# Alex-McAvoy/Light-Graph-Convolutional-Recommendation-Algorithm-based-on-Hybrid-Spreading

Hardware: AMD Instinct MI355X
Metric: propagation edges/sec + full-catalog top-K recs/sec, 1/2/4/8 MI355X (higher is better)
Workload: dtype f32; 1 GPU; c5-d64; users=1000000, items=1000000, interactions=100000000, directed_nnz=200000000, dim=64, layers=3, parallelism=row-shard x1 + RCCL all-gather per layer

## Files before the change

### light-graph-convolutional-recommendation-algorithm-based-on-hybrid-spreading_amd/csrc/spread_tiled.hip

```cpp
#include <stdio.h>
#include <stdlib.h>

#include "common.h"

#ifndef LG_REFERENCE_PATHS
#define LG_REFERENCE_PATHS 0
#endif
#if LG_REFERENCE_PATHS
#include "lgcnhs_ref.h"
#endif

namespace lg {

typedef float f32x4 __attribute__((ext_vector_type(4)));

constexpr uint32_t kHdrV = 0x80000000u;
constexpr uint32_t kHdrOvf = 0x40000000u;
constexpr uint32_t kHdrSlow = 0x20000000u;
constexpr uint32_t kHdrPtr = 0x1FFFFFFFu;
constexpr uint32_t kEntV = 0x80000000u;
constexpr uint32_t kRunDense = 0x80000000u;
constexpr int kLineSlots = 31;
constexpr int kLineEnts = 7;
constexpr int kInvTab = 512;
// ... 948 lines not shown
          while (need) {
            const int u = __ffsll((long long)need) - 1;
            need &= need - 1;
            compact_user(g, u, lim);
          }
        }
      }
    }
  };

  float af0[Q], af1[Q], af2[Q], af3[Q];
  double f0[NG][4], f1[NG][4], f2[NG][4], f3[NG][4];
  load_step(0, af0, f0);
  load_step(16, af1, f1);
  load_step(32, af2, f2);
  for (int it = 0;; it += 64) {
    load_step(it + 48, af3, f3);
    process(it, af0, f0);
    if (it + 16 >= n_cols) break;
    load_step(it + 64, af0, f0);
    process(it + 16, af1, f1);
    if (it + 32 >= n_cols) break;
    load_step(it + 80, af1, f1);
    process(it + 32, af2, f2);
    if (it + 48 >= n_cols) break;
    load_step(it + 96, af2, f2);
    process(it + 48, af3, f3);
    if (it + 64 >= n_cols) break;
  }

  wave_sync();
#pragma unroll
  for (int g = 0; g < NG; ++g) {
    for (int u = 0; u < 16; ++u) {
      const int64_t r = ubase + g * 16 + u;
      if (r >= n_rows) break;
      if (!__shfl((int)dirty[g], u)) continue;
      compact_user(g, u, lim_end);
      const int nc = __shfl(cnt[g], u);
      for (int e = lane; e < k; e += 64) {
        const double v = e < nc ? cs[wave][g][u][e] : neg_inf<double>();
        const bool ok = e < nc && v != neg_inf<double>();
        io_val[r * k + e] = ok ? v : neg_inf<double>();
        io_idx[r * k + e] = ok ? ci[wave][g][u][e] : -1;
      }
      wave_sync();
    }
  }
}

#endif

constexpr int MODE_F = 0, MODE_TOPK = 1;
constexpr int kWalkQ = 8;
constexpr int kBatchRows = 8 * kWalkQ;
constexpr int kOvfList = kBatchRows > 64 ? kBatchRows : 64;
constexpr int kDecodePhase = 4;
constexpr int kQPre = 8;
static_assert(kWalkQ % kDecodePhase == 0, "decode phase must divide the batch's line loads");

struct WalkArgs {
  const int64_t *user_rowptr;
  const int32_t *user_items;
  const double *ra_edge;
  int64_t n_users;
  const uint4 *lines;
  const uint4 *ovf;
  int32_t null_row;
  int32_t item_begin, tile, width;
  const double *rbeta;
  const double *g_inv;
  double *F;
  int64_t ldf;
  const float *eu, *ei;
  const float *gb;
  int32_t nch;
  const uint8_t *qb;
  int32_t qstride;
  const int64_t *ex_rowptr;
  const int32_t *ex_col;
  int64_t *ex_cur;
  int k, first;
  double *io_val;
  int64_t *io_idx;
};

__host__ __device__ constexpr int acc_cols(int tile) { return (tile + 511) / 512 * 512; }

template <int MODE, int D, int M>
__host__ __device__ constexpr size_t walk_wave_bytes(int tile) {
  return ((size_t)acc_cols(tile) * 8 + (size_t)kOvfList * 12 + 15) & ~(size_t)15;
}
__host__ __device__ constexpr size_t walk_shared_bytes(int tile) {
  return (size_t)kInvTab * 8 + 16 * 8 + (size_t)((tile + 1) & ~1) * 8 + 64 * 8;
}


typedef __attribute__((address_space(3))) double lds_f64;
__device__ __forceinline__ double slot_inv_fast(uint32_t s) {
  return *(const lds_f64 *)(uintptr_t)(s >> 13);
}
__device__ __forceinline__ void slot_add_nobranch(uint32_t acc_base, uint32_t dummy, uint32_t s,
                                                  double v) {
  uint32_t addr;
  asm("v_mad_u32_u16 %0, %1, 8, %2" : "=v"(addr) : "v"(s), "v"(acc_base));
  addr = s ? addr : dummy;
  __hip_atomic_fetch_add((lds_f64 *)(uintptr_t)addr, v, __ATOMIC_RELAXED,
                         __HIP_MEMORY_SCOPE_WORKGROUP);
}

__device__ __forceinline__ double slot_inv(uint32_t s, const double *s_inv,
                                           const double *__restrict__ g_inv) {
  const uint32_t c = s >> 16;
  const bool far = c >= (uint32_t)kInvTab;
  const double inv = s_inv[far ? 0u : c];
  if (__builtin_expect(__ballot(far) != 0, 0)) {
    const double g = __builtin_nontemporal_load(g_inv + (far ? c : 0u));
    return far ? g : inv;
  }
  return inv;
}

__device__ __forceinline__ void add_unit(double *acc, uint4 w, bool head, double ra,
                                         const double *s_inv, const double *__restrict__ g_inv) {
  const bool isv = !head && (w.x & kEntV);
  const uint32_t sx = head ? 0u : w.x;
  const uint32_t py = isv ? 0u : w.y, pz = isv ? 0u : w.z, pw = isv ? 0u : w.w;
  const double i0 = slot_inv(isv ? 0u : sx, s_inv, g_inv);
  const double v0 = (isv ? __hiloint2double((int)w.z, (int)w.y) : i0) * ra;
  const double v1 = slot_inv(py, s_inv, g_inv) * ra;
  const double v2 = slot_inv(pz, s_inv, g_inv) * ra;
  const double v3 = slot_inv(pw, s_inv, g_inv) * ra;
  if (sx) lds_add(acc, sx & 0xFFFFu, v0);
  if (py) lds_add(acc, py & 0xFFFFu, v1);
  if (pz) lds_add(acc, pz & 0xFFFFu, v2);
  if (pw) lds_add(acc, pw & 0xFFFFu, v3);
}

__device__ __forceinline__ void add_unit_v(double *acc, uint4 w, double ra) {
  if (w.x & kEntV) lds_add(acc, w.x & 0xFFFFu, __hiloint2double((int)w.z, (int)w.y) * ra);
}
__device__ __forceinline__ void add_unit_d(double *acc, uint4 w, int q, double ra) {
  const double a = __hiloint2double((int)w.y, (int)w.x), b = __hiloint2double((int)w.w, (int)w.z);
  if (a != 0.0) lds_add(acc, (uint32_t)(2 * q), a * ra);
  if (b != 0.0) lds_add(acc, (uint32_t)(2 * q + 1), b * ra);
}

__device__ __forceinline__ void add_slot_fast(double *acc, uint32_t s, double ra,
                                              const double *s_inv) {
  const double inv = s_inv[s >> 16];
  if (s) lds_add(acc, s & 0xFFFFu, inv * ra);
}

struct Batch {
  int32_t u, r0, r1, e;
  bool first;
  int32_t xc, xh;
};

struct UState {
  int lid0, lid1;
  double lv0, lv1;
  float gb;
  uint32_t q[kQPre];
  int32_t xw;
};

template <int MODE, int D, int M, bool SEED = false>
__global__ __launch_bounds__(512) void k_tile_walk(WalkArgs a) {
  constexpr int Q = kWalkQ;
  extern __shared__ double lds[];
  const int nw = blockDim.x / 64;
  const int wave = __builtin_amdgcn_readfirstlane(threadIdx.x / 64);
  const int lane = lane_id();
  const int gh = lane & 7;
  const int grow = lane >> 3;
  const uint32_t hmask = gh == 0 ? 0u : 0xFFFFFFFFu;
  const int tile = a.tile;
  double *s_inv = lds;
  double *s_red = s_inv + kInvTab;
  double *s_rb = s_red + 16;
  double *s_rbc = s_rb + ((tile + 1) & ~1);
  char *mine = reinterpret_cast<char *>(s_rbc + 64) +
               (size_t)wave * walk_wave_bytes<MODE, D, M>(tile);
  double *acc = reinterpret_cast<double *>(mine);
  const uint32_t acc_base = (uint32_t)(uintptr_t)(lds_f64 *)acc;
  const uint32_t dummy_addr = acc_base + 8u * (uint32_t)(acc_cols(tile) + lane);
  double *ovl_ra = acc + acc_cols(tile);
  uint32_t *ovl_ent = reinterpret_cast<uint32_t *>(ovl_ra + kOvfList);

  for (int c = threadIdx.x; c < kInvTab; c += blockDim.x) s_inv[c] = a.g_inv[c];
  double rmax = 0.0;
  for (int j = threadIdx.x; j < tile; j += blockDim.x) {
    const double rb = j < a.width ? a.rbeta[a.item_begin + j] : 0.0;
    s_rb[j] = rb;
    rmax = fmax(rmax, rb);
  }
#pragma unroll
  for (int o = 32; o > 0; o >>= 1) rmax = fmax(rmax, __shfl_xor(rmax, o));
  if (lane == 0) s_red[wave] = rmax;
  for (int j = lane; j < acc_cols(tile); j += 64) acc[j] = 0.0;
  __syncthreads();
  if (MODE == MODE_TOPK && D > 0) {
    for (int c = wave; 64 * c < tile && c < 64; c += nw) {
      double m = s_rb[64 * c + lane < tile ? 64 * c + lane : 0];
#pragma unroll
      for (int o = 32; o > 0; o >>= 1) m = fmax(m, __shfl_xor(m, o));
      if (lane == 0) s_rbc[c] = m;
    }
    __syncthreads();
  }
  rmax = 0.0;
  for (int w = 0; w < nw; ++w) rmax = fmax(rmax, s_red[w]);
  const double rscale = rmax * (1.0 + 0x1p-50);

  const int64_t G = (int64_t)gridDim.x * nw;
  const int64_t n_users = a.n_users;
  const int64_t u_first = (int64_t)blockIdx.x * nw + wave;
  if (u_first >= n_users) return;

  const bool has_ex = MODE == MODE_TOPK && a.ex_rowptr != nullptr;
  int32_t uq = (int32_t)u_first;
  int32_t pr = 0, px = 0;
  auto pre_load = [&]() __attribute__((always_inline)) {
    const int64_t uu = uq < n_users ? uq : n_users - 1;
    pr = reinterpret_cast<const int32_t *>(a.user_rowptr)[2 * (uu + (lane & 1))];
    if (has_ex) {
      const int64_t *p = (lane & 1) ? a.ex_rowptr + uu + 1 : a.ex_cur + uu;
      px = *reinterpret_cast<const int32_t *>(p);
    }
  };
  pre_load();
  auto new_user = [&]() __attribute__((always_inline)) {
    const int32_t bq = __builtin_amdgcn_readlane(pr, 0), eq = __builtin_amdgcn_readlane(pr, 1);
    const int32_t xcq = has_ex ? __builtin_amdgcn_readlane(px, 0) : 0;
    const int32_t xhq = has_ex ? __builtin_amdgcn_readlane(px, 1) : 0;
    Batch y{uq, bq, bq + kBatchRows < eq ? bq + kBatchRows : eq, eq, true, xcq, xhq};
    uq += (int32_t)G;
    return y;
  };
  const Batch kEnd{(int32_t)n_users, 0, 0, 0, false, 0, 0};
  auto next_batch = [&](const Batch &x) __attribute__((always_inline)) {
    if (x.u >= n_users) return kEnd;
    if (x.r1 < x.e) {
      Batch y{x.u, x.r1, x.r1 + kBatchRows < x.e ? x.r1 + kBatchRows : x.e, x.e, false, x.xc,
              x.xh};
      return y;
    }
    if (x.u + G >= n_users) return kEnd;
    return new_user();
  };
  const __amdgpu_buffer_rsrc_t r_lines = __builtin_amdgcn_make_buffer_rsrc(
      (void *)a.lines, 0, (int)((uint32_t)(a.null_row + 1) * 128u), 0x00020000);
  auto load_ids = [&](const Batch &x, int32_t (&it)[Q]) __attribute__((always_inline)) {
    {
      const __amdgpu_buffer_rsrc_t rs = __builtin_amdgcn_make_buffer_rsrc(
          (void *)(a.user_items + x.r0), 0, (int)((x.r1 - x.r0) * 4), 0x00020000);
#pragma unroll
      for (int q = 0; q < Q; ++q)
        it[q] = (int32_t)__builtin_amdgcn_raw_buffer_load_b32(rs, (uint32_t)(grow * 4 + 32 * q),
                                                              0, 0);
    }
  };
  auto load_rows = [&](const Batch &x, const int32_t (&it)[Q], uint4 (&w)[Q], double (&ra)[Q])
      __attribute__((always_inline)) {
    const int nr = (int)(x.r1 - x.r0);
    const __amdgpu_buffer_rsrc_t rr = __builtin_amdgcn_make_buffer_rsrc(
        (void *)(a.ra_edge + x.r0), 0, nr * 8, 0x00020000);
#pragma unroll
    for (int q = 0; q < Q; ++q) {
      const bool in = 8 * q + grow < nr;
      const uint32_t row = in ? (uint32_t)it[q] : (uint32_t)a.null_row;
      const auto v = __builtin_amdgcn_raw_buffer_load_b128(r_lines, row * 128u + 16u * gh, 0, 0);
      w[q] = uint4{v[0], v[1], v[2], v[3]};
      const auto d = __builtin_amdgcn_raw_buffer_load_b64(rr, (uint32_t)(grow * 8 + 64 * q), 0, 0);
      ra[q] = __builtin_bit_cast(double, d);
    }
  };

  constexpr bool kTwo = M > 2;
  const bool has_qb = MODE == MODE_TOPK && D > 0 && a.qb != nullptr;
  auto load_state = [&](const Batch &x, UState &st) __attribute__((always_inline)) {
    if constexpr (MODE == MODE_TOPK) {
      const int k = a.k;
      const int64_t us = x.u < n_users ? x.u : n_users - 1;
      const int *idx32 = reinterpret_cast<const int *>(a.io_idx);
      const int e0 = lane < k ? lane : k - 1;
      st.lid0 = idx32[2 * (us * k + e0)];
      st.lv0 = a.io_val[us * k + e0];
      if constexpr (kTwo) {
        const int e1 = 64 + lane < k ? 64 + lane : k - 1;
        st.lid1 = idx32[2 * (us * k + e1)];
        st.lv1 = a.io_val[us * k + e1];
      }
      if constexpr (D > 0) {
        st.gb = a.gb[us * a.nch + (lane < a.nch ? lane : 0)];
        const __amdgpu_buffer_rsrc_t rq = __builtin_amdgcn_make_buffer_rsrc(
            has_qb ? (void *)(a.qb + us * a.qstride) : (void *)a.lines, 0,
            has_qb ? a.qstride : 0, 0x00020000);
#pragma unroll
        for (int kk = 0; kk < kQPre; ++kk)
          st.q[kk] = __builtin_amdgcn_raw_buffer_load_b32(rq, (uint32_t)(4 * lane + 256 * kk), 0, 0);
      }
      const int32_t nx = x.xh - x.xc;
      const __amdgpu_buffer_rsrc_t rx = __builtin_amdgcn_make_buffer_rsrc(
          has_ex ? (void *)(a.ex_col + x.xc) : (void *)a.lines, 0,
          has_ex ? (int)(4 * (nx < 64 ? nx : 64)) : 0, 0x00020000);
      st.xw = (int32_t)__builtin_amdgcn_raw_buffer_load_b32(rx, (uint32_t)(4 * lane), 0, 0);
    }
  };

  auto decode = [&](const Batch &x, uint4 (&w)[Q], const double (&ra)[Q])
      __attribute__((always_inline)) {
#ifdef LG_WALK_PROBE
    if (LG_WALK_PROBE == 2) {
      uint32_t h = 0;
#pragma unroll
      for (int q = 0; q < Q; ++q) h ^= w[q].x ^ w[q].y ^ w[q].z ^ w[q].w ^ (uint32_t)ra[q];
      if (h == 0x12345678u && lane == 64) acc[0] = 1.0;
      return;
    }
#endif
    uint32_t hdr = 0;
#pragma unroll
    for (int q = 0; q < Q; ++q) hdr |= w[q].x & ~hmask;
    const bool slow = __ballot(hdr & kHdrSlow) != 0;
    const bool ovf = __ballot(hdr & kHdrOvf) != 0;
    if (!slow) {
      constexpr int H = kDecodePhase;
      const int nr = (int)(x.r1 - x.r0);
#pragma unroll
      for (int q0 = 0; q0 < Q; q0 += H) {
        if (8 * q0 >= nr) break;
        double inv[H][4];
#pragma unroll
        for (int q = 0; q < H; ++q) {
          if (8 * (q0 + q) >= nr) break;
          inv[q][0] = slot_inv_fast(w[q0 + q].x & hmask);
          inv[q][1] = slot_inv_fast(w[q0 + q].y);
          inv[q][2] = slot_inv_fast(w[q0 + q].z);
          inv[q][3] = slot_inv_fast(w[q0 + q].w);
        }
#pragma unroll
        for (int q = 0; q < H; ++q) {
          if (8 * (q0 + q) >= nr) break;
          const uint32_t sv[4] = {w[q0 + q].x & hmask, w[q0 + q].y, w[q0 + q].z, w[q0 + q].w};
#pragma unroll
          for (int t = 0; t < 4; ++t)
            slot_add_nobranch(acc_base, dummy_addr, sv[t], inv[q][t] * ra[q0 + q]);
        }
      }
    } else {
#pragma unroll
      for (int q = 0; q < Q; ++q) add_unit(acc, w[q], gh == 0, ra[q], s_inv, a.g_inv);
    }
    if (ovf) {
      int nov = 0;
#pragma unroll
      for (int q = 0; q < Q; ++q) {
        const bool o = gh == 0 && (w[q].x & kHdrOvf);
        const uint64_t bal = __ballot(o);
        if (o) {
          const int p = nov + __popcll(bal & lanemask_lt());
          ovl_ent[p] = w[q].x & (kHdrPtr | kHdrV);
          ovl_ra[p] = ra[q];
        }
        nov += __popcll(bal);
      }
      wave_sync();
      for (int t0 = 0; t0 < nov; t0 += 4) {
        uint4 y4[4];
        uint32_t ou4[4];
        double r4[4];
        bool v4[4];
#pragma unroll
        for (int j = 0; j < 4; ++j) {
          const bool in = t0 + j < nov;
          const uint32_t e = ovl_ent[in ? t0 + j : t0];
          v4[j] = (e & kHdrV) != 0;
          ou4[j] = e & kHdrPtr;
          r4[j] = ovl_ra[in ? t0 + j : t0];
          y4[j] = a.ovf[(int64_t)ou4[j] + lane];
        }
#pragma unroll
        for (int j = 0; j < 4; ++j) {
          if (t0 + j >= nov) continue;
          const uint32_t n0 = (uint32_t)__shfl((int)y4[j].x, 0);
          const bool dn = (n0 & kRunDense) != 0;
          const uint32_t n = n0 & ~kRunDense;
          if (lane == 0 || (uint32_t)lane > n) y4[j] = uint4{0u, 0u, 0u, 0u};
          if (dn) add_unit_d(acc, y4[j], lane - 1, r4[j]);
          else if (v4[j]) add_unit_v(acc, y4[j], r4[j]);
          else add_unit(acc, y4[j], false, r4[j], s_inv, a.g_inv);
          for (uint32_t c = 64; c <= n; c += 256) {
            uint4 z[4];
#pragma unroll
            for (int p = 0; p < 4; ++p) {
              const uint32_t cc = c + 64 * p + lane;
              z[p] = cc <= n ? a.ovf[(int64_t)ou4[j] + cc] : uint4{0u, 0u, 0u, 0u};
            }
#pragma unroll
            for (int p = 0; p < 4; ++p) {
              if (c + 64 * p > n) break;
              if (dn) add_unit_d(acc, z[p], (int)(c + 64 * p) + lane - 1, r4[j]);
              else if (v4[j]) add_unit_v(acc, z[p], r4[j]);
              else add_unit(acc, z[p], false, r4[j], s_inv, a.g_inv);
            }
          }
        }
      }
      wave_sync();
    }
  };

  auto finish_user = [&](const Batch &x, UState &st) __attribute__((always_inline)) {
    const int64_t u = x.u;
    wave_sync();
#ifdef LG_WALK_PROBE
    if (LG_WALK_PROBE == 1) {
      for (int j = 2 * lane; j < acc_cols(tile); j += 128)
        *reinterpret_cast<double2 *>(acc + j) = double2{0.0, 0.0};
      wave_sync();
      return;
    }
#endif
    if constexpr (MODE == MODE_F) {
      double *row = a.F + u * a.ldf;
      for (int j = lane; j < tile; j += 64) {
        __builtin_nontemporal_store(acc[j] * s_rb[j], row + j);
        acc[j] = 0.0;
      }
    } else {
      const int k = a.k;
      const bool ok0 = !a.first && lane < k && st.lid0 >= 0;
      double L0 = ok0 ? st.lv0 : neg_inf<double>();
      int I0 = ok0 ? st.lid0 : kPadId;
      double L1 = neg_inf<double>();
      int I1 = kPadId;
      if constexpr (kTwo) {
        const bool ok1 = !a.first && 64 + lane < k && st.lid1 >= 0;
        L1 = ok1 ? st.lv1 : neg_inf<double>();
        I1 = ok1 ? st.lid1 : kPadId;
      }
      const float gbv = st.gb;
      uint32_t (&qr)[kQPre] = st.q;
      if (!has_qb) {
#pragma unroll
        for (int kk = 0; kk < kQPre; ++kk) qr[kk] = 0xFFFFFFFFu;
      }
      int64_t xpos = x.xc;
      const int64_t xhi = x.xh;
      int32_t xw = has_ex && xpos + lane < xhi ? st.xw : 0x7fffffff;
      auto kth = [&](double &tv, int &ti) __attribute__((always_inline)) {
        if (!kTwo || k <= 64) {
          tv = __shfl(L0, k - 1);
          ti = __shfl(I0, k - 1);
        } else {
          tv = __shfl(L1, k - 65);
          ti = __shfl(I1, k - 65);
        }
      };
      double tau;
      int tau_id;
      kth(tau, tau_id);
      bool dirty = a.first != 0;
      auto insert1 = [&](double v, int id) __attribute__((always_inline)) {
        if (!before(v, id, tau, tau_id)) return;
        dirty = true;
        int pos = __popcll(__ballot(before(L0, I0, v, id)));
        if constexpr (kTwo) pos += __popcll(__ballot(before(L1, I1, v, id)));
        const double up0 = __shfl_up(L0, 1);
        const int iu0 = __shfl_up(I0, 1);
        if constexpr (kTwo) {
          const double up1 = __shfl_up(L1, 1);
          const int iu1 = __shfl_up(I1, 1);
          const double c0 = __shfl(L0, 63);
          const int ic0 = __shfl(I0, 63);
          const int p1 = 64 + lane;
          const double n1 = p1 > pos ? (lane == 0 ? c0 : up1) : (p1 == pos ? v : L1);
          const int m1 = p1 > pos ? (lane == 0 ? ic0 : iu1) : (p1 == pos ? id : I1);
          L1 = p1 < k ? n1 : neg_inf<double>();
          I1 = p1 < k ? m1 : kPadId;
        }
        L0 = lane > pos ? up0 : (lane == pos ? v : L0);
        I0 = lane > pos ? iu0 : (lane == pos ? id : I0);
        if (lane >= k) { L0 = neg_inf<double>(); I0 = kPadId; }
        kth(tau, tau_id);
      };
      const int32_t lim = a.item_begin + a.width;
      if (has_ex) {
        for (;;) {
          const bool in = xw < lim;
          if (in && xw >= a.item_begin) acc[xw - a.item_begin] = neg_inf<double>();
          const int nin = __popcll(__ballot(in));
          xpos += nin;
          if (nin < 64) break;
          xw = xpos + lane < xhi ? a.ex_col[xpos + lane] : 0x7fffffff;
        }
        if (lane == 0) a.ex_cur[u] = xpos;
      }
      wave_sync();
      int ncand = 0;
      double *cq_f = ovl_ra;
      uint32_t *cq_j = ovl_ent;
      auto flush = [&]() __attribute__((always_inline)) {
#ifdef LG_WALK_PROBE
        if (LG_WALK_PROBE == 3) {
          wave_sync();
          for (int mm = 0; mm < ncand; ++mm) insert1(cq_f[mm], a.item_begin + (int)cq_j[mm]);
          ncand = 0;
          wave_sync();
          return;
        }
#endif
        if constexpr (D > 0) {
          constexpr int Qd = D / 4;
          constexpr int H = Qd < 16 ? Qd : 16;
          wave_sync();
          const int m = lane & 15, g = lane >> 4;
          for (int b0 = 0; b0 < ncand; b0 += 16) {
            const int nb = ncand - b0 < 16 ? ncand - b0 : 16;
            const int ci = b0 + (m < nb ? m : 0);
            const float *ir = a.ei + (int64_t)(a.item_begin + (int)cq_j[ci]) * D + g * Qd;
            const float *ur = a.eu + u * D + g * Qd;
            f32x4 sc4 = f32x4{0.f, 0.f, 0.f, 0.f};
#pragma unroll
            for (int h0 = 0; h0 < Qd; h0 += H) {
              float av[H], bv[H];
              load_frag<H>(ir + h0, av);
              load_frag<H>(ur + h0, bv);
#pragma unroll
              for (int s = 0; s < H; ++s)
                sc4 = __builtin_amdgcn_mfma_f32_16x16x4f32(av[s], bv[s], sc4, 0, 0, 0);
            }
            for (int mm = 0; mm < nb; ++mm) {
              const float e = (mm & 3) == 0 ? sc4[0] : (mm & 3) == 1 ? sc4[1]
                            : (mm & 3) == 2 ? sc4[2] : sc4[3];
              const float sc = __shfl(e, 16 * (mm >> 2));
              insert1((double)sc * cq_f[b0 + mm], a.item_begin + (int)cq_j[b0 + mm]);
            }
          }
          ncand = 0;
          wave_sync();
        }
      };
      double thr_s = tau / rscale;
      double sc_v = 0.0, bq_v = 0.0;
      if constexpr (D > 0) {
        const double gp = (double)fmaxf(gbv, 0.f);
        sc_v = s_rbc[lane < a.nch ? lane : 0] * (1.0 + 0x1p-50) * gp * (1.0 / 255.0);
        bq_v = gp * (1.0 / 255.0) * (1.0 + 0x1p-50);
      }
      bool seeded = false;
      double t_hi = 0.0;
      if constexpr (SEED && D > 0 && !kTwo) {
        if (tau == neg_inf<double>()) {
          auto read8 = [&](int c0, double (&sv)[8]) __attribute__((always_inline)) {
#pragma unroll
            for (int hh = 0; hh < 2; ++hh)
#pragma unroll
              for (int pp = 0; pp < 2; ++pp) {
                const int j = c0 + 256 * hh + 4 * lane + 2 * pp;
                const double2 x = *reinterpret_cast<const double2 *>(acc + j);
                sv[4 * hh + 2 * pp] = x.x;
                sv[4 * hh + 2 * pp + 1] = x.y;
              }
            if (c0 + 512 > a.width) {
#pragma unroll
              for (int t = 0; t < 8; ++t) {
                const int j = c0 + 256 * (t >> 2) + 4 * lane + (t & 3);
                if (j >= a.width) sv[t] = neg_inf<double>();
              }
            }
          };
          auto qsel = [&](int i) __attribute__((always_inline)) {
            uint32_t v = 0xFFFFFFFFu;
#pragma unroll
            for (int x = 0; x < kQPre; ++x) v = i == x ? qr[x] : v;
            return v;
          };
          auto bound = [&](int c0, int t, double svt, uint32_t qa, uint32_t qb2)
              __attribute__((always_inline)) {
            const double sc = __shfl(sc_v, ((c0 + 256 * (t >> 2) + 4 * lane) >> 6) & 63);
            const uint32_t qq = t < 4 ? qa : qb2;
            const double qv = (double)((qq >> (8 * (t & 3))) & 0xFFu);
            return svt * qv * sc;
          };
          double lmax = neg_inf<double>();
#pragma unroll 1
          for (int c0 = 0; c0 < a.width; c0 += 512) {
            double sv[8];
            read8(c0, sv);
            const uint32_t qa = qsel(c0 >> 8), qb2 = qsel((c0 >> 8) + 1);
#pragma unroll
            for (int t = 0; t < 8; ++t) {
              const double bt = bound(c0, t, sv[t], qa, qb2);
              lmax = bt > lmax ? bt : lmax;
            }
          }
          double v = lmax;
#pragma unroll
          for (int sz = 2; sz <= 64; sz <<= 1)
#pragma unroll
            for (int st2 = sz >> 1; st2 > 0; st2 >>= 1) {
              const double o = __shfl_xor(v, st2);
              const bool keep_max = ((lane & sz) == 0) == ((lane & st2) == 0);
              v = keep_max ? (o > v ? o : v) : (o < v ? o : v);
            }
          t_hi = __shfl(v, k - 1);
          seeded = true;
#pragma unroll 1
          for (int c0 = 0; c0 < a.width; c0 += 512) {
            double sv[8];
            read8(c0, sv);
            const uint32_t qa = qsel(c0 >> 8), qb2 = qsel((c0 >> 8) + 1);
            uint32_t mask = 0;
#pragma unroll
            for (int t = 0; t < 8; ++t) {
              const double bt = bound(c0, t, sv[t], qa, qb2);
              mask |= bt >= t_hi && bt > neg_inf<double>() ? 1u << t : 0u;
            }
            while (__ballot(mask != 0)) {
              const bool has = mask != 0;
              const int t = has ? __ffs(mask) - 1 : 0;
              mask &= mask - 1;
              double sx = sv[0];
#pragma unroll
              for (int x = 1; x < 8; ++x) sx = t == x ? sv[x] : sx;
              const int j = c0 + 256 * (t >> 2) + 4 * lane + (t & 3);
              const double f = has ? sx * s_rb[has ? j : 0] : -1.0;
              const uint64_t bal = __ballot(has);
              const int nb = __popcll(bal);
              if (ncand + nb > kOvfList) flush();
              if (has) {
                const int p = ncand + __popcll(bal & lanemask_lt());
                cq_f[p] = f;
                cq_j[p] = (uint32_t)j;
              }
              ncand += nb;
              if (ncand >= 16) flush();
            }
          }
          if (ncand) flush();
        }
      }
      const double2 zero2{0.0, 0.0};
      for (int c0 = 0; c0 < a.width; c0 += 512) {
        const uint32_t qa = qr[0], qb2 = qr[1];
#pragma unroll
        for (int k = 0; k + 2 < kQPre; ++k) qr[k] = qr[k + 2];
        qr[kQPre - 2] = 0xFFFFFFFFu;
        qr[kQPre - 1] = 0xFFFFFFFFu;
        double sv[8];
#pragma unroll
        for (int hh = 0; hh < 2; ++hh)
#pragma unroll
          for (int pp = 0; pp < 2; ++pp) {
            const int j = c0 + 256 * hh + 4 * lane + 2 * pp;
            const double2 x = *reinterpret_cast<const double2 *>(acc + j);
            *reinterpret_cast<double2 *>(acc + j) = zero2;
            sv[4 * hh + 2 * pp] = x.x;
            sv[4 * hh + 2 * pp + 1] = x.y;
          }
        if (c0 + 512 > a.width) {
#pragma unroll
          for (int t = 0; t < 8; ++t) {
            const int j = c0 + 256 * (t >> 2) + 4 * lane + (t & 3);
            if (j >= a.width) sv[t] = neg_inf<double>();
          }
        }
        double sc0 = 0.0, sc1 = 0.0;
        if constexpr (D > 0) {
          sc0 = __shfl(sc_v, ((c0 + 4 * lane) >> 6) & 63);
          sc1 = __shfl(sc_v, ((c0 + 256 + 4 * lane) >> 6) & 63);
        }
        uint32_t mask = 0;
#pragma unroll
        for (int t = 0; t < 8; ++t) {
          bool pre;
          if constexpr (D > 0) {
            const uint32_t qq = t < 4 ? qa : qb2;
            const double qv = (double)((qq >> (8 * (t & 3))) & 0xFFu);
            const double b = sv[t] * qv * (t < 4 ? sc0 : sc1);
            pre = b > tau && !(seeded && b >= t_hi && b > neg_inf<double>());
          } else {
            pre = sv[t] > thr_s;
          }
          mask |= pre ? 1u << t : 0u;
        }
        while (__ballot(mask != 0)) {
          const bool has = mask != 0;
          const int t = has ? __ffs(mask) - 1 : 0;
          mask &= mask - 1;
          double s = sv[0];
#pragma unroll
          for (int x = 1; x < 8; ++x) s = t == x ? sv[x] : s;
          const int j = c0 + 256 * (t >> 2) + 4 * lane + (t & 3);
          const double f = has ? s * s_rb[has ? j : 0] : -1.0;
          if constexpr (D > 0) {
            const uint32_t qq = t < 4 ? qa : qb2;
            const double bq = (double)((qq >> (8 * (t & 3))) & 0xFFu) *
                              __shfl(bq_v, (j >> 6) & 63);
            const bool cand = has && bq * f > tau;
            const uint64_t bal = __ballot(cand);
            if (bal) {
              const int nb = __popcll(bal);
              if (ncand + nb > kOvfList) flush();
              if (cand) {
                const int p = ncand + __popcll(bal & lanemask_lt());
                cq_f[p] = f;
                cq_j[p] = (uint32_t)j;
              }
              ncand += nb;
              if (ncand >= 16 || tau == neg_inf<double>()) flush();
            }
          } else {
            uint64_t bal = __ballot(has && before(f, a.item_begin + j, tau, tau_id));
            while (bal) {
              const int l = __ffsll((long long)bal) - 1;
              bal &= bal - 1;
              insert1(__shfl(f, l), a.item_begin + __shfl(j, l));
            }
            thr_s = tau / rscale;
          }
        }
      }
      if (ncand) flush();
      if (dirty) {
        if (lane < k) {
          a.io_val[u * k + lane] = I0 != kPadId ? L0 : neg_inf<double>();
          a.io_idx[u * k + lane] = I0 != kPadId ? I0 : -1;
        }
        if (kTwo && 64 + lane < k) {
          a.io_val[u * k + 64 + lane] = I1 != kPadId ? L1 : neg_inf<double>();
          a.io_idx[u * k + 64 + lane] = I1 != kPadId ? I1 : -1;
        }
      }
      wave_sync();
    }
  };

  int32_t it2[Q];
  uint4 w0[Q], w1[Q];
  double ra0[Q], ra1[Q];
  UState s0, s1;
  Batch c = new_user();
  pre_load();
  load_ids(c, it2);
  load_rows(c, it2, w0, ra0);
  load_state(c, s0);
  Batch d = next_batch(c);
  pre_load();
  load_ids(d, it2);
  load_rows(d, it2, w1, ra1);
  load_state(d, s1);
  Batch n2 = next_batch(d);
  pre_load();
  load_ids(n2, it2);
  auto step = [&](uint4 (&wc)[Q], double (&rc)[Q], UState &sc) __attribute__((always_inline)) {
    if constexpr (MODE == MODE_TOPK) {
      asm volatile("" : "+v"(sc.lid0), "+v"(sc.lv0), "+v"(sc.xw));
      if constexpr (kTwo) asm volatile("" : "+v"(sc.lid1), "+v"(sc.lv1));
      if constexpr (D > 0) {
        asm volatile("" : "+v"(sc.gb));
#pragma unroll
        for (int kk = 0; kk < kQPre; ++kk) asm volatile("" : "+v"(sc.q[kk]));
      }
    }
    decode(c, wc, rc);
    if (c.r1 >= c.e) finish_user(c, sc);
    load_rows(n2, it2, wc, rc);
    load_state(n2, sc);
    const Batch n3 = next_batch(n2);
    pre_load();
    load_ids(n3, it2);
    c = d;
    d = n2;
    n2 = n3;
    return c.u < n_users;
  };
  for (;;) {
    if (!step(w0, ra0, s0)) break;
    if (!step(w1, ra1, s1)) break;
  }
}

#if LG_REFERENCE_PATHS
template <int D, bool VEC>
static void launch_tile_topk_v(int M, const double *F, int64_t ldf, int64_t n_rows, int32_t j0,
                               int32_t n_cols, const float *eu, const float *ei,
                               const int64_t *ex_rowptr, const int32_t *ex_col, int drop,
                               int k, int first, double *io_val, int64_t *io_idx,
                               hipStream_t s) {
  if (M == 1 && k <= 24 && !first) {
    const unsigned b = (unsigned)((n_rows + 63) / 64);
    k_tile_topk<D, 2, 1, VEC, 40><<<b, 128, 0, s>>>(F, ldf, n_rows, j0, n_cols, eu, ei,
                                                    ex_rowptr, ex_col, drop, k, first, io_val,
                                                    io_idx);
  } else if (M == 1) {
    const unsigned b = (unsigned)((n_rows + 63) / 64);
    k_tile_topk<D, 2, 1, VEC, 64><<<b, 128, 0, s>>>(F, ldf, n_rows, j0, n_cols, eu, ei,
                                                    ex_rowptr, ex_col, drop, k, first, io_val,
                                                    io_idx);
  } else if (M == 2) {
    const unsigned b = (unsigned)((n_rows + 31) / 32);
    k_tile_topk<D, 1, 2, VEC, 128><<<b, 128, 0, s>>>(F, ldf, n_rows, j0, n_cols, eu, ei,
                                                     ex_rowptr, ex_col, drop, k, first, io_val,
                                                     io_idx);
  } else {
    const unsigned b = (unsigned)((n_rows + 31) / 32);
    k_tile_topk<D, 1, 4, VEC, 256><<<b, 128, 0, s>>>(F, ldf, n_rows, j0, n_cols, eu, ei,
                                                     ex_rowptr, ex_col, drop, k, first, io_val,
                                                     io_idx);
  }
}

template <int D>
static void launch_tile_topk(int M, const double *F, int64_t ldf, int64_t n_rows, int32_t j0,
                             int32_t n_cols, const float *eu, const float *ei,
                             const int64_t *ex_rowptr, const int32_t *ex_col, int drop, int k,
                             int first, double *io_val, int64_t *io_idx, hipStream_t s) {
  const bool vec = ldf >= ((int64_t)n_cols + 15) / 16 * 16 && (ldf % 2) == 0 &&
                   ((uintptr_t)F % 16) == 0;
  if (vec)
    launch_tile_topk_v<D, true>(M, F, ldf, n_rows, j0, n_cols, eu, ei, ex_rowptr, ex_col, drop, k,
                             first, io_val, io_idx, s);
  else
    launch_tile_topk_v<D, false>(M, F, ldf, n_rows, j0, n_cols, eu, ei, ex_rowptr, ex_col, drop, k,
                             first, io_val, io_idx, s);
}

#endif

template <int M>
__global__ __launch_bounds__(256) void k_lists_merge_f64(const double *__restrict__ in_val,
                                                         const int64_t *__restrict__ in_idx,
                                                         int n_lists, int64_t n_rows, int k,
                                                         double *__restrict__ out_val,
                                                         int64_t *__restrict__ out_idx) {
  constexpr int CAP = 64 * M;
  __shared__ double cs[4][CAP];
  __shared__ int ci[4][CAP];
  const int wave = threadIdx.x / 64;
  const int lane = lane_id();
  const int64_t row = (int64_t)blockIdx.x * 4 + wave;
  if (row >= n_rows) return;
  int cnt = 0;
  double tau = neg_inf<double>();
  int tau_id = kPadId;
  for (int s = 0; s < n_lists; ++s) {
    const int64_t base = ((int64_t)s * n_rows + row) * k;
    for (int e0 = 0; e0 < k; e0 += 64) {
      const int e = e0 + lane;
      double v = neg_inf<double>();
      int id = -1;
      if (e < k) {
        const int64_t x = in_idx[base + e];
        if (x >= 0) {
          v = in_val[base + e];
          id = (int)x;
        }
      }
      const bool cand = id >= 0 && before(v, id, tau, tau_id);
      const uint64_t bal = __ballot(cand);
      const int pos = cnt + __popcll(bal & lanemask_lt());
      if (cand) {
        cs[wave][pos] = v;
        ci[wave][pos] = id;
      }
      cnt += __popcll(bal);
      if (cnt > CAP - 64) {
        wave_sync();
        cnt = wave_compact<double, M>(cs[wave], ci[wave], cnt, k, tau, tau_id);
      }
    }
  }
  wave_sync();
  const int nc = wave_compact<double, M>(cs[wave], ci[wave], cnt, k, tau, tau_id);
  for (int e = lane; e < k; e += 64) {
    out_val[row * k + e] = e < nc ? cs[wave][e] : neg_inf<double>();
    out_idx[row * k + e] = e < nc ? ci[wave][e] : -1;
  }
}

}

using namespace lg;

extern "C" int lg_spread_tile_seek(const int64_t *user_rowptr, const int32_t *user_items,
                                   int64_t n_users, int32_t item_begin, int64_t *cur,
                                   lg_stream_t stream) {
  LG_REQUIRE(user_rowptr && cur && n_users >= 0 && item_begin >= 0,
             "lg_spread_tile_seek: bad arguments");
  if (n_users == 0) return LG_OK;
  k_tile_seek<<<dim3((unsigned)((n_users + 255) / 256)), dim3(256), 0, (hipStream_t)stream>>>(
      user_rowptr, user_items, n_users, item_begin, cur);
  return launch_status("lg_spread_tile_seek");
}

extern "C" int lg_topk_lists_merge_f64(const double *in_val, const int64_t *in_idx,
                                       int32_t n_lists, int64_t n_rows, int32_t k,
                                       double *out_val, int64_t *out_idx, lg_stream_t stream) {
  LG_REQUIRE(n_lists >= 1 && n_rows >= 0, "lg_topk_lists_merge_f64: bad sizes");
  LG_REQUIRE(k >= 1 && k <= 128, "lg_topk_lists_merge_f64: k=%d not in [1,128]", k);
  LG_REQUIRE(n_rows == 0 || (in_val && in_idx && out_val && out_idx),
             "lg_topk_lists_merge_f64: NULL argument");
  if (n_rows == 0) return LG_OK;
  const dim3 grid((unsigned)((n_rows + 3) / 4));
  hipStream_t s = (hipStream_t)stream;
  if (k <= 64)
    k_lists_merge_f64<2><<<grid, dim3(256), 0, s>>>(in_val, in_idx, n_lists, n_rows, k, out_val,
                                                    out_idx);
  else
    k_lists_merge_f64<4><<<grid, dim3(256), 0, s>>>(in_val, in_idx, n_lists, n_rows, k, out_val,
                                                    out_idx);
  return launch_status("lg_topk_lists_merge_f64");
}

extern "C" int lg_hybrid_recip_f64(const double *k_item, int64_t n_items, double lambda,
                                   double *ra, double *rb, lg_stream_t stream) {
  LG_REQUIRE(k_item && ra && rb && n_items >= 0, "lg_hybrid_recip_f64: bad arguments");
  if (n_items == 0) return LG_OK;
  k_hybrid_recip<<<dim3((unsigned)((n_items + 255) / 256)), dim3(256), 0,
                   (hipStream_t)stream>>>(k_item, n_items, lambda, ra, rb);
  return launch_status("lg_hybrid_recip_f64");
}

extern "C" int lg_inv_degree_f64(const int64_t *rowptr, int64_t n_rows, double *inv,
                                 lg_stream_t stream) {
  LG_REQUIRE(rowptr && inv && n_rows >= 0, "lg_inv_degree_f64: bad arguments");
  if (n_rows == 0) return LG_OK;
  k_inv_degree<<<dim3((unsigned)((n_rows + 255) / 256)), dim3(256), 0, (hipStream_t)stream>>>(
      rowptr, n_rows, inv);
  return launch_status("lg_inv_degree_f64");
}

#if LG_REFERENCE_PATHS
// ... 361 lines not shown
```

Before: 27.67 billion edge-layers/s.

## Issue walk-kernel loads via inline asm with explicit vmcnt waits for software pipelining

Replaces compiler-generated buffer/global loads in the tiled walk kernel with inline-asm loads and a single explicit s_waitcnt vmcnt(0) per step. The aim is to stop the compiler from inserting conservative waits, so the next batch's row and state loads stay in flight while the current batch is decoded. Per-user top-K state is now loaded only for a user's last batch, which skips redundant state loads on intermediate batches. The cost is manual s_nop hazard gaps and full-drain waits that could serialize more than before, plus correctness risk from hand-managed register pinning.

```diff
diff --git a/light-graph-convolutional-recommendation-algorithm-based-on-hybrid-spreading_amd/csrc/spread_tiled.hip b/light-graph-convolutional-recommendation-algorithm-based-on-hybrid-spreading_amd/csrc/spread_tiled.hip
--- a/light-graph-convolutional-recommendation-algorithm-based-on-hybrid-spreading_amd/csrc/spread_tiled.hip
+++ b/light-graph-convolutional-recommendation-algorithm-based-on-hybrid-spreading_amd/csrc/spread_tiled.hip
@@ -1124,6 +1124,41 @@
   if (s) lds_add(acc, s & 0xFFFFu, inv * ra);
 }
 
+typedef uint32_t u32x4 __attribute__((ext_vector_type(4)));
+__device__ __forceinline__ void pipe_sgpr_gap() { asm volatile("s_nop 4"); }
+__device__ __forceinline__ uint32_t pipe_load_b32(__amdgpu_buffer_rsrc_t rs, uint32_t voff,
+                                                  int imm) {
+  uint32_t x;
+  asm volatile("buffer_load_dword %0, %1, %2, 0 offen offset:%3"
+               : "=v"(x) : "v"(voff), "s"(rs), "i"(imm));
+  return x;
+}
+__device__ __forceinline__ double pipe_load_b64(__amdgpu_buffer_rsrc_t rs, uint32_t voff,
+                                                int imm) {
+  double x;
+  asm volatile("buffer_load_dwordx2 %0, %1, %2, 0 offen offset:%3"
+               : "=v"(x) : "v"(voff), "s"(rs), "i"(imm));
+  return x;
+}
+__device__ __forceinline__ u32x4 pipe_load_b128(__amdgpu_buffer_rsrc_t rs, uint32_t voff) {
+  u32x4 x;
+  asm volatile("buffer_load_dwordx4 %0, %1, %2, 0 offen" : "=v"(x) : "v"(voff), "s"(rs));
+  return x;
+}
+__device__ __forceinline__ uint32_t pipe_gload_b32(const void *p) {
+  uint32_t x;
+  asm volatile("global_load_dword %0, %1, off" : "=v"(x) : "v"(p));
+  return x;
+}
+__device__ __forceinline__ double pipe_gload_b64(const void *p) {
+  double x;
+  asm volatile("global_load_dwordx2 %0, %1, off" : "=v"(x) : "v"(p));
+  return x;
+}
+__device__ __forceinline__ void pipe_wait() { asm volatile("s_waitcnt vmcnt(0)"); }
+template <class T>
+__device__ __forceinline__ void pipe_pin(T &x) { asm volatile("" : "+v"(x)); }
+
 struct Batch {
   int32_t u, r0, r1, e;
   bool first;
@@ -1131,11 +1166,11 @@
 };
 
 struct UState {
-  int lid0, lid1;
+  uint32_t lid0, lid1;
   double lv0, lv1;
-  float gb;
+  uint32_t gb;
   uint32_t q[kQPre];
-  int32_t xw;
+  uint32_t xw;
 };
 
 template <int MODE, int D, int M, bool SEED = false>
@@ -1193,20 +1228,20 @@
 
   const bool has_ex = MODE == MODE_TOPK && a.ex_rowptr != nullptr;
   int32_t uq = (int32_t)u_first;
-  int32_t pr = 0, px = 0;
+  uint32_t pr = 0, px = 0;
   auto pre_load = [&]() __attribute__((always_inline)) {
     const int64_t uu = uq < n_users ? uq : n_users - 1;
-    pr = reinterpret_cast<const int32_t *>(a.user_rowptr)[2 * (uu + (lane & 1))];
+    pr = pipe_gload_b32(reinterpret_cast<const int32_t *>(a.user_rowptr) + 2 * (uu + (lane & 1)));
     if (has_ex) {
       const int64_t *p = (lane & 1) ? a.ex_rowptr + uu + 1 : a.ex_cur + uu;
-      px = *reinterpret_cast<const int32_t *>(p);
+      px = pipe_gload_b32(p);
     }
   };
-  pre_load();
   auto new_user = [&]() __attribute__((always_inline)) {
-    const int32_t bq = __builtin_amdgcn_readlane(pr, 0), eq = __builtin_amdgcn_readlane(pr, 1);
-    const int32_t xcq = has_ex ? __builtin_amdgcn_readlane(px, 0) : 0;
-    const int32_t xhq = has_ex ? __builtin_amdgcn_readlane(px, 1) : 0;
+    const int32_t bq = __builtin_amdgcn_readlane((int)pr, 0);
+    const int32_t eq = __builtin_amdgcn_readlane((int)pr, 1);
+    const int32_t xcq = has_ex ? __builtin_amdgcn_readlane((int)px, 0) : 0;
+    const int32_t xhq = has_ex ? __builtin_amdgcn_readlane((int)px, 1) : 0;
     Batch y{uq, bq, bq + kBatchRows < eq ? bq + kBatchRows : eq, eq, true, xcq, xhq};
     uq += (int32_t)G;
     return y;
@@ -1224,29 +1259,27 @@
   };
   const __amdgpu_buffer_rsrc_t r_lines = __builtin_amdgcn_make_buffer_rsrc(
       (void *)a.lines, 0, (int)((uint32_t)(a.null_row + 1) * 128u), 0x00020000);
-  auto load_ids = [&](const Batch &x, int32_t (&it)[Q]) __attribute__((always_inline)) {
-    {
-      const __amdgpu_buffer_rsrc_t rs = __builtin_amdgcn_make_buffer_rsrc(
-          (void *)(a.user_items + x.r0), 0, (int)((x.r1 - x.r0) * 4), 0x00020000);
-#pragma unroll
-      for (int q = 0; q < Q; ++q)
-        it[q] = (int32_t)__builtin_amdgcn_raw_buffer_load_b32(rs, (uint32_t)(grow * 4 + 32 * q),
-                                                              0, 0);
-    }
+  auto load_ids = [&](const Batch &x, uint32_t (&it)[Q]) __attribute__((always_inline)) {
+    const int nr = (int)(x.r1 - x.r0);
+    const __amdgpu_buffer_rsrc_t rs = __builtin_amdgcn_make_buffer_rsrc(
+        (void *)(a.user_items + x.r0), 0, nr * 4, 0x00020000);
+    pipe_sgpr_gap();
+#pragma unroll
+    for (int q = 0; q < Q; ++q)
+      it[q] = pipe_load_b32(rs, (uint32_t)(grow * 4), 32 * q);
   };
-  auto load_rows = [&](const Batch &x, const int32_t (&it)[Q], uint4 (&w)[Q], double (&ra)[Q])
+  auto load_rows = [&](const Batch &x, const uint32_t (&it)[Q], u32x4 (&w)[Q], double (&ra)[Q])
       __attribute__((always_inline)) {
     const int nr = (int)(x.r1 - x.r0);
     const __amdgpu_buffer_rsrc_t rr = __builtin_amdgcn_make_buffer_rsrc(
         (void *)(a.ra_edge + x.r0), 0, nr * 8, 0x00020000);
+    pipe_sgpr_gap();
 #pragma unroll
     for (int q = 0; q < Q; ++q) {
       const bool in = 8 * q + grow < nr;
-      const uint32_t row = in ? (uint32_t)it[q] : (uint32_t)a.null_row;
-      const auto v = __builtin_amdgcn_raw_buffer_load_b128(r_lines, row * 128u + 16u * gh, 0, 0);
-      w[q] = uint4{v[0], v[1], v[2], v[3]};
-      const auto d = __builtin_amdgcn_raw_buffer_load_b64(rr, (uint32_t)(grow * 8 + 64 * q), 0, 0);
-      ra[q] = __builtin_bit_cast(double, d);
+      const uint32_t row = in ? it[q] : (uint32_t)a.null_row;
+      w[q] = pipe_load_b128(r_lines, row * 128u + 16u * gh);
+      ra[q] = pipe_load_b64(rr, (uint32_t)(grow * 8), 64 * q);
     }
   };
 
@@ -1258,31 +1291,33 @@
       const int64_t us = x.u < n_users ? x.u : n_users - 1;
       const int *idx32 = reinterpret_cast<const int *>(a.io_idx);
       const int e0 = lane < k ? lane : k - 1;
-      st.lid0 = idx32[2 * (us * k + e0)];
-      st.lv0 = a.io_val[us * k + e0];
+      st.lid0 = pipe_gload_b32(idx32 + 2 * (us * k + e0));
+      st.lv0 = pipe_gload_b64(a.io_val + us * k + e0);
       if constexpr (kTwo) {
         const int e1 = 64 + lane < k ? 64 + lane : k - 1;
-        st.lid1 = idx32[2 * (us * k + e1)];
-        st.lv1 = a.io_val[us * k + e1];
+        st.lid1 = pipe_gload_b32(idx32 + 2 * (us * k + e1));
+        st.lv1 = pipe_gload_b64(a.io_val + us * k + e1);
       }
       if constexpr (D > 0) {
-        st.gb = a.gb[us * a.nch + (lane < a.nch ? lane : 0)];
+        st.gb = pipe_gload_b32(a.gb + us * a.nch + (lane < a.nch ? lane : 0));
         const __amdgpu_buffer_rsrc_t rq = __builtin_amdgcn_make_buffer_rsrc(
             has_qb ? (void *)(a.qb + us * a.qstride) : (void *)a.lines, 0,
             has_qb ? a.qstride : 0, 0x00020000);
+        pipe_sgpr_gap();
 #pragma unroll
         for (int kk = 0; kk < kQPre; ++kk)
-          st.q[kk] = __builtin_amdgcn_raw_buffer_load_b32(rq, (uint32_t)(4 * lane + 256 * kk), 0, 0);
+          st.q[kk] = pipe_load_b32(rq, (uint32_t)(4 * lane), 256 * kk);
       }
       const int32_t nx = x.xh - x.xc;
       const __amdgpu_buffer_rsrc_t rx = __builtin_amdgcn_make_buffer_rsrc(
           has_ex ? (void *)(a.ex_col + x.xc) : (void *)a.lines, 0,
           has_ex ? (int)(4 * (nx < 64 ? nx : 64)) : 0, 0x00020000);
-      st.xw = (int32_t)__builtin_amdgcn_raw_buffer_load_b32(rx, (uint32_t)(4 * lane), 0, 0);
+      pipe_sgpr_gap();
+      st.xw = pipe_load_b32(rx, (uint32_t)(4 * lane), 0);
     }
   };
 
-  auto decode = [&](const Batch &x, uint4 (&w)[Q], const double (&ra)[Q])
+  auto decode = [&](const Batch &x, const u32x4 (&w)[Q], const double (&ra)[Q])
       __attribute__((always_inline)) {
 #ifdef LG_WALK_PROBE
     if (LG_WALK_PROBE == 2) {
@@ -1324,7 +1359,8 @@
       }
     } else {
 #pragma unroll
-      for (int q = 0; q < Q; ++q) add_unit(acc, w[q], gh == 0, ra[q], s_inv, a.g_inv);
+      for (int q = 0; q < Q; ++q)
+        add_unit(acc, uint4{w[q].x, w[q].y, w[q].z, w[q].w}, gh == 0, ra[q], s_inv, a.g_inv);
     }
     if (ovf) {
       int nov = 0;
@@ -1404,17 +1440,17 @@
       }
     } else {
       const int k = a.k;
-      const bool ok0 = !a.first && lane < k && st.lid0 >= 0;
+      const bool ok0 = !a.first && lane < k && (int)st.lid0 >= 0;
       double L0 = ok0 ? st.lv0 : neg_inf<double>();
-      int I0 = ok0 ? st.lid0 : kPadId;
+      int I0 = ok0 ? (int)st.lid0 : kPadId;
       double L1 = neg_inf<double>();
       int I1 = kPadId;
       if constexpr (kTwo) {
-        const bool ok1 = !a.first && 64 + lane < k && st.lid1 >= 0;
+        const bool ok1 = !a.first && 64 + lane < k && (int)st.lid1 >= 0;
         L1 = ok1 ? st.lv1 : neg_inf<double>();
-        I1 = ok1 ? st.lid1 : kPadId;
-      }
-      const float gbv = st.gb;
+        I1 = ok1 ? (int)st.lid1 : kPadId;
+      }
+      const float gbv = __uint_as_float(st.gb);
       uint32_t (&qr)[kQPre] = st.q;
       if (!has_qb) {
 #pragma unroll
@@ -1422,7 +1458,7 @@
       }
       int64_t xpos = x.xc;
       const int64_t xhi = x.xh;
-      int32_t xw = has_ex && xpos + lane < xhi ? st.xw : 0x7fffffff;
+      int32_t xw = has_ex && xpos + lane < xhi ? (int32_t)st.xw : 0x7fffffff;
       auto kth = [&](double &tv, int &ti) __attribute__((always_inline)) {
         if (!kTwo || k <= 64) {
           tv = __shfl(L0, k - 1);
@@ -1712,37 +1748,67 @@
     }
   };
 
-  int32_t it2[Q];
-  uint4 w0[Q], w1[Q];
+  uint32_t it2[Q] = {};
+  u32x4 w0[Q], w1[Q];
   double ra0[Q], ra1[Q];
-  UState s0, s1;
+  UState s0 = {}, s1 = {};
+  auto landed = [&](u32x4 (&w)[Q], double (&ra)[Q], UState &st) __attribute__((always_inline)) {
+    pipe_wait();
+    pipe_pin(pr);
+    pipe_pin(px);
+#pragma unroll
+    for (int q = 0; q < Q; ++q) {
+      pipe_pin(it2[q]);
+      pipe_pin(w[q]);
+      pipe_pin(ra[q]);
+    }
+    if constexpr (MODE == MODE_TOPK) {
+      pipe_pin(st.lid0);
+      pipe_pin(st.lv0);
+      pipe_pin(st.xw);
+      if constexpr (kTwo) {
+        pipe_pin(st.lid1);
+        pipe_pin(st.lv1);
+      }
+      if constexpr (D > 0) {
+        pipe_pin(st.gb);
+#pragma unroll
+        for (int kk = 0; kk < kQPre; ++kk) pipe_pin(st.q[kk]);
+      }
+    }
+  };
+  auto load_last = [&](const Batch &x, UState &st) __attribute__((always_inline)) {
+    if (x.r1 >= x.e && x.u < n_users) load_state(x, st);
+  };
+#pragma unroll
+  for (int q = 0; q < Q; ++q) {
+    w0[q] = w1[q] = u32x4{0u, 0u, 0u, 0u};
+    ra0[q] = ra1[q] = 0.0;
+  }
+  pre_load();
+  landed(w0, ra0, s0);
   Batch c = new_user();
   pre_load();
   load_ids(c, it2);
+  landed(w0, ra0, s0);
   load_rows(c, it2, w0, ra0);
-  load_state(c, s0);
+  load_last(c, s0);
   Batch d = next_batch(c);
   pre_load();
   load_ids(d, it2);
+  landed(w0, ra0, s0);
   load_rows(d, it2, w1, ra1);
-  load_state(d, s1);
+  load_last(d, s1);
   Batch n2 = next_batch(d);
   pre_load();
   load_ids(n2, it2);
-  auto step = [&](uint4 (&wc)[Q], double (&rc)[Q], UState &sc) __attribute__((always_inline)) {
-    if constexpr (MODE == MODE_TOPK) {
-      asm volatile("" : "+v"(sc.lid0), "+v"(sc.lv0), "+v"(sc.xw));
-      if constexpr (kTwo) asm volatile("" : "+v"(sc.lid1), "+v"(sc.lv1));
-      if constexpr (D > 0) {
-        asm volatile("" : "+v"(sc.gb));
-#pragma unroll
-        for (int kk = 0; kk < kQPre; ++kk) asm volatile("" : "+v"(sc.q[kk]));
-      }
-    }
+  auto step = [&](u32x4 (&wc)[Q], double (&rc)[Q], UState &sc, u32x4 (&wn)[Q], double (&rn)[Q],
+                  UState &sn) __attribute__((always_inline)) {
     decode(c, wc, rc);
     if (c.r1 >= c.e) finish_user(c, sc);
+    landed(wn, rn, sn);
     load_rows(n2, it2, wc, rc);
-    load_state(n2, sc);
+    load_last(n2, sc);
     const Batch n3 = next_batch(n2);
     pre_load();
     load_ids(n3, it2);
@@ -1752,9 +1818,10 @@
     return c.u < n_users;
   };
   for (;;) {
-    if (!step(w0, ra0, s0)) break;
-    if (!step(w1, ra1, s1)) break;
-  }
+    if (!step(w0, ra0, s0, w1, ra1, s1)) break;
+    if (!step(w1, ra1, s1, w0, ra0, s0)) break;
+  }
+  pipe_wait();
 }
 
 #if LG_REFERENCE_PATHS
```

Result: no change. 27.67 billion edge-layers/s (median of 2 runs) (-0.0%).
